# yanielc/medical-vision-textural-bias

Hardware: AMD Instinct MI355X
Metric: BraTS 4ch 240^3 vols/sec filtered+train-step @1/2/4/8 GPU; filter HBM GB/s (higher is better)
Workload: dtype f32

## Files before the change

medical-vision-textural-bias_amd/csrc/conv_up.hip:

```cpp
#include <hip/hip_runtime.h>

#include <cstdlib>
#include <type_traits>

#include "num_cu.h"
#include "texbias.h"

namespace {

typedef float f2v __attribute__((ext_vector_type(2)));
typedef float f32x4 __attribute__((ext_vector_type(4)));
typedef const __attribute__((address_space(4))) float* cfloat_p;
typedef const __attribute__((address_space(4))) f2v* cf2v_p;

template <int B, int N, class F>
__device__ __forceinline__ void static_for(F&& f) {
  if constexpr (B < N) {
    f(std::integral_constant<int, B>{});
    static_for<B + 1, N>(f);
  }
}

struct S2Args {
  const float* in;
  const float* K;
  const float* bias;
  float* out;
  int Do, Ho, Wo, Di, Hi, Wi;
  int ZS, zlen, nyb;
  int PX, RR;
};

template <int CIN, int MOUT, int TY, int WV, int NTH = 256>
__global__ __launch_bounds__(NTH) void k_conv_s2_fewin(S2Args a) {
  static_assert(MOUT % 2 == 0, "packed output pairs");
  constexpr int NHALF = NTH / 256, MP = MOUT / 2 / NHALF;
  constexpr int NR = 2 * TY + 1;
  extern __shared__ __attribute__((aligned(16))) float smem[];
  const int tid = (int)threadIdx.x;
  constexpr int PX = 4 * WV + 12, SS = CIN * NR * PX;
  float* ring = smem;
  for (int i = tid; i < 3 * SS; i += NTH) ring[i] = 0.f;
  int b = (int)blockIdx.x;
  const int zs = b % a.ZS;
  b /= a.ZS;
  const int yb = b % a.nyb, n = b / a.nyb;
  const int y0 = yb * TY;
  const int z0 = zs * a.zlen, z1 = min(a.Do, z0 + a.zlen);
  const int Di = a.Di, Hi = a.Hi, Wi = a.Wi;
  const int64_t iplane = (int64_t)Hi * Wi, iplane4 = iplane / 4;
  const float4* inb = reinterpret_cast<const float4*>(a.in + (int64_t)n * CIN * Di * iplane);
  const int W4 = Wi >> 2;
  constexpr int NL = (CIN * NR * WV + NTH - 1) / NTH;
  int gof[NL], lof[NL];
#pragma unroll
  for (int j = 0; j < NL; ++j) {
    const int i = tid + NTH * j;
    const int q = i % W4, t = i / W4, r = t % NR, c = t / NR;
    const int yi = 2 * y0 - 1 + r;
    const bool ok = c < CIN && yi >= 0 && yi < Hi;
    gof[j] = ok ? (int)((int64_t)c * Di * iplane4 + ((int64_t)yi * Wi + 4 * q) / 4) : -1;
    lof[j] = (c * NR + r) * PX + 4 + 4 * q;
  }
  float4 ra[NL], rb[NL];
  auto load = [&](int zi, float4 (&r)[NL]) {
    const bool in = zi >= 0 && zi < Di;
    const float4* src = inb + (int64_t)(in ? zi : 0) * iplane4;
#pragma unroll
    for (int j = 0; j < NL; ++j) {
      r[j] = src[gof[j] < 0 ? 0 : gof[j]];
    }
  };
  auto store = [&](int zi, const float4 (&r)[NL]) {
    float* d = ring + ((zi + 3) % 3) * SS;
    const bool in = zi >= 0 && zi < Di;
#pragma unroll
    for (int j = 0; j < NL; ++j)
      if (gof[j] >= 0) *reinterpret_cast<float4*>(d + lof[j]) = in ? r[j] : make_float4(0.f, 0.f, 0.f, 0.f);
  };
  __syncthreads();
  load(2 * z0 - 1, ra);
  store(2 * z0 - 1, ra);
  load(2 * z0, ra);
  load(2 * z0 + 1, rb);
  const int pt = tid & 255, mh = __builtin_amdgcn_readfirstlane(tid >> 8);
  const int Wo = a.Wo, oy = pt / Wo, ox = pt - oy * Wo;
  const bool act = oy < TY && y0 + oy < a.Ho;
  const int roff = (2 * oy) * PX + 2 * ox + 3;
  f2v bias2[MP];
#pragma unroll
  for (int mm = 0; mm < MP; ++mm) {
    const int m = mh * MP + mm;
    bias2[mm] = a.bias ? f2v{a.bias[2 * m], a.bias[2 * m + 1]} : f2v{0.f, 0.f};
  }
  const int64_t oplane = (int64_t)a.Ho * Wo;
  float* outb = a.out + (int64_t)n * MOUT * a.Do * oplane + (int64_t)(y0 + oy) * Wo + ox;
  constexpr bool LATE = NTH == 256;
  f2v pend[MP];
  auto put = [&](int zp) {
    float* o = outb + (int64_t)zp * oplane;
#pragma unroll
    for (int mm = 0; mm < MP; ++mm) {
      const int m = mh * MP + mm;
      o[(int64_t)(2 * m) * a.Do * oplane] = pend[mm].x;
      o[(int64_t)(2 * m + 1) * a.Do * oplane] = pend[mm].y;
    }
  };
  for (int z = z0; z < z1; ++z) {
    store(2 * z, ra);
    store(2 * z + 1, rb);
    __syncthreads();
    if (LATE || z + 1 < z1) {
      load(2 * z + 2, ra);
      load(2 * z + 3, rb);
    }
    if (LATE && act && z > z0) put(z - 1);
    if (act) {
      float v[CIN * 27];
#pragma unroll
      for (int tz = 0; tz < 3; ++tz) {
        const float* sl = ring + ((2 * z - 1 + tz + 3) % 3) * SS + roff;
#pragma unroll
        for (int c = 0; c < CIN; ++c)
#pragma unroll
          for (int ty = 0; ty < 3; ++ty)
#pragma unroll
            for (int tx = 0; tx < 3; ++tx) v[c * 27 + tz * 9 + ty * 3 + tx] = sl[(c * NR + ty) * PX + tx];
      }
      constexpr int KC = CIN * 27, NP = MP * KC, BT = 16, NB = (NP + BT - 1) / BT;
      const cf2v_p kp = (cf2v_p)(cfloat_p)a.K + mh * NP;
      f2v kb[2][BT];
      auto kload = [&](int b, f2v (&k)[BT]) {
#pragma unroll
        for (int i = 0; i < BT; ++i)
          if (b * BT + i < NP) k[i] = kp[b * BT + i];
      };
      kload(0, kb[0]);
      f2v acc = bias2[0];
      static_for<0, NB>([&](auto bc) {
        constexpr int b = decltype(bc)::value;
        __builtin_amdgcn_sched_barrier(0);
        __builtin_amdgcn_s_waitcnt(0xc07f);
        __builtin_amdgcn_sched_barrier(0);
        if (b + 1 < NB) kload(b + 1, kb[(b + 1) & 1]);
        __builtin_amdgcn_sched_barrier(0);
#pragma unroll
        for (int i = 0; i < BT; ++i) {
          const int p = b * BT + i, mm = p / KC, k = p - mm * KC;
          if (p < NP) {
            if (k == 0) acc = bias2[mm];
            acc = __builtin_elementwise_fma(f2v{v[k], v[k]}, kb[b & 1][i], acc);
            if (k == KC - 1) {
              if (LATE) {
                pend[mm] = acc;
              } else {
                const int m = mh * MP + mm;
                float* o = outb + (int64_t)z * oplane;
                o[(int64_t)(2 * m) * a.Do * oplane] = acc.x;
                o[(int64_t)(2 * m + 1) * a.Do * oplane] = acc.y;
              }
            }
          }
        }
      });
    }
    __syncthreads();
  }
  if (LATE && act && z1 > z0) put(z1 - 1);
}

struct TArgs {
  const float* x;
  const float* W;
  const float* bias;
  float* y;
  int Cin, Di, Hi, Wi;
  int ZS, zlen, nyb;
  int PX, CS;
};

template <int MO, int TY, int WV, int NTH = 256, int U = 1>
__global__ __launch_bounds__(NTH) void k_convT_fewout(TArgs a) {
  extern __shared__ __attribute__((aligned(16))) float smem[];
  const int tid = (int)threadIdx.x;
  constexpr int PX = 4 * WV + 8, CS = (TY + 1) * PX;
  const int Cin = a.Cin, SS = Cin * CS;
  float* ring = smem;
  for (int i = tid; i < 2 * SS; i += NTH) ring[i] = 0.f;
  const cfloat_p wg = (cfloat_p)a.W;
  int b = (int)blockIdx.x;
  const int zs = b % a.ZS;
  b /= a.ZS;
  const int yb = b % a.nyb, n = b / a.nyb;
  const int y0 = yb * TY;
  const int Di = a.Di, Hi = a.Hi, Wi = a.Wi;
  const int z0 = zs * a.zlen, z1 = min(Di, z0 + a.zlen);
  const int64_t iplane = (int64_t)Hi * Wi, iplane4 = iplane / 4;
  const float4* xb = reinterpret_cast<const float4*>(a.x + (int64_t)n * Cin * Di * iplane);
  const int W4 = Wi >> 2;
  constexpr int NL = (32 * (TY + 1) * WV + NTH - 1) / NTH;
  const int nitem = Cin * (TY + 1) * W4;
  int gof[NL], lof[NL];
#pragma unroll
  for (int j = 0; j < NL; ++j) {
    const int i = tid + NTH * j;
    const int q = i % W4, t = i / W4, r = t % (TY + 1), c = t / (TY + 1);
    const int yi = y0 + r;
    const bool ok = i < nitem && yi < Hi;
    gof[j] = ok ? (int)((int64_t)c * Di * iplane4 + ((int64_t)yi * Wi + 4 * q) / 4) : -1;
    lof[j] = c * CS + r * PX + 4 + 4 * q;
  }
  float4 rg[NL];
  auto load = [&](int zi) {
    const bool in = zi < Di;
    const float4* src = xb + (int64_t)(in ? zi : 0) * iplane4;
#pragma unroll
    for (int j = 0; j < NL; ++j) {
      rg[j] = src[gof[j] < 0 ? 0 : gof[j]];
    }
  };
  auto store = [&](int zi) {
    float* d = ring + (zi & 1) * SS;
    const bool in = zi < Di;
#pragma unroll
    for (int j = 0; j < NL; ++j)
      if (gof[j] >= 0) *reinterpret_cast<float4*>(d + lof[j]) = in ? rg[j] : make_float4(0.f, 0.f, 0.f, 0.f);
  };
  __syncthreads();
  load(z0);
  store(z0);
  load(z0 + 1);
  const int jy = tid / Wi, jx = tid - jy * Wi;
  const bool act = jy < TY && y0 + jy < Hi;
  const int roff = jy * PX + jx + 4;
  const int Ho = 2 * Hi, Wo = 2 * Wi, Do = 2 * Di;
  const int64_t oplane = (int64_t)Ho * Wo;
  float bia[MO];
#pragma unroll
  for (int m = 0; m < MO; ++m) bia[m] = a.bias ? a.bias[m] : 0.f;
  float* yb0 = a.y + (int64_t)n * MO * Do * oplane + (int64_t)(2 * (y0 + jy)) * Wo + 2 * jx;
  for (int z = z0; z < z1; ++z) {
    store(z + 1);
    __syncthreads();
    if (z + 1 < z1) load(z + 2);
    float acc[MO][2][2][2];
#pragma unroll
    for (int m = 0; m < MO; ++m)
#pragma unroll
      for (int p = 0; p < 8; ++p) acc[m][p >> 2][(p >> 1) & 1][p & 1] = bia[m];
    if (act) {
      const float* s0 = ring + (z & 1) * SS + roff;
      const float* s1 = ring + ((z + 1) & 1) * SS + roff;
#pragma unroll U
      for (int c = 0; c < Cin; ++c) {
        float v[2][2][2];
        v[0][0][0] = s0[c * CS];
        v[0][0][1] = s0[c * CS + 1];
        v[0][1][0] = s0[c * CS + PX];
        v[0][1][1] = s0[c * CS + PX + 1];
        v[1][0][0] = s1[c * CS];
        v[1][0][1] = s1[c * CS + 1];
        v[1][1][0] = s1[c * CS + PX];
        v[1][1][1] = s1[c * CS + PX + 1];
        const cfloat_p wc = wg + c * MO * 27;
#pragma unroll
        for (int m = 0; m < MO; ++m) {
          const cfloat_p wk = wc + m * 27;
#pragma unroll
          for (int pz = 0; pz < 2; ++pz)
#pragma unroll
            for (int py = 0; py < 2; ++py)
#pragma unroll
              for (int px = 0; px < 2; ++px) {
                float s = acc[m][pz][py][px];
#pragma unroll
                for (int dz = 0; dz <= pz; ++dz)
#pragma unroll
                  for (int dy = 0; dy <= py; ++dy)
#pragma unroll
                    for (int dx = 0; dx <= px; ++dx) {
                      const int tz = pz ? (dz ? 0 : 2) : 1, ty = py ? (dy ? 0 : 2) : 1, tx = px ? (dx ? 0 : 2) : 1;
                      s = fmaf(v[dz][dy][dx], wk[tz * 9 + ty * 3 + tx], s);
                    }
                acc[m][pz][py][px] = s;
              }
        }
      }
#pragma unroll
      for (int m = 0; m < MO; ++m)
#pragma unroll
        for (int pz = 0; pz < 2; ++pz)
#pragma unroll
          for (int py = 0; py < 2; ++py) {
            float* o = yb0 + ((int64_t)m * Do + 2 * z + pz) * oplane + (int64_t)py * Wo;
            *reinterpret_cast<float2*>(o) = make_float2(acc[m][pz][py][0], acc[m][pz][py][1]);
          }
    }
    __syncthreads();
  }
}

int zseg(int D, int base, int per_cu, int fill) {
  const int slots = per_cu * tb::num_cu();
  int best = 1 << 30, zl = D;
  for (int l = D; l >= 1; --l) {
    const int zs = (D + l - 1) / l, rounds = (base * zs + slots - 1) / slots, cost = rounds * (l + fill);
    if (cost < best) best = cost, zl = l;
  }
  return zl;
}

template <int CIN, int MOUT, int WV>
int launch_s2(S2Args& a, size_t lds, int N, hipStream_t st) {
  constexpr int TY = 3;
  constexpr int NT = (CIN == 4 && MOUT == 32) ? 512 : 256;
  auto kern = k_conv_s2_fewin<CIN, MOUT, TY, WV, NT>;
  if (hipFuncSetAttribute(reinterpret_cast<const void*>(kern), hipFuncAttributeMaxDynamicSharedMemorySize, 163840) !=
      hipSuccess)
    return TB_ERR_HIP;
  const int per_cu = lds <= 81920 ? 2 : 1;
  a.zlen = zseg(a.Do, N * a.nyb, per_cu, 1);
  a.ZS = (a.Do + a.zlen - 1) / a.zlen;
  hipLaunchKernelGGL(kern, dim3((unsigned)(N * a.nyb * a.ZS)), dim3(NT), lds, st, a);
  return hipGetLastError() == hipSuccess ? TB_OK : TB_ERR_HIP;
}

}

int tb_conv3d_s2_fewin_f32(const float* in, const float* K, const float* bias, float* out, int N, int Cin, int Mout,
                           int Do, int Ho, int Wo, void* stream) {
  if (!in || !K || !out || N < 1 || Do < 1 || Ho < 1 || Wo < 1) return TB_ERR_INVALID_ARG;
  if (Cin < 1 || Cin > 4 || (Mout != 16 && Mout != 32) || 3 * Wo > 256 || (2 * Wo) % 4 != 0 || 2 * Wo > 256 ||
      (reinterpret_cast<uintptr_t>(in) & 15) != 0)
    return TB_ERR_UNSUPPORTED_SIZE;
  constexpr int TY = 3;
  S2Args a{};
  a.in = in, a.K = K, a.bias = bias, a.out = out;
  a.Do = Do, a.Ho = Ho, a.Wo = Wo, a.Di = 2 * Do, a.Hi = 2 * Ho, a.Wi = 2 * Wo;
  const bool wide = a.Wi > 160;
  a.PX = 4 * (wide ? 64 : 40) + 12;
  a.RR = 2 * TY + 1;
  a.nyb = (Ho + TY - 1) / TY;
  const size_t lds = (size_t)4 * 3 * Cin * a.RR * a.PX;
  if (lds > 163840) return TB_ERR_UNSUPPORTED_SIZE;
  hipStream_t st = reinterpret_cast<hipStream_t>(stream);
#define TB_S2(CI, MO)                                                                                  \
  if (Cin == CI && Mout == MO) return wide ? launch_s2<CI, MO, 64>(a, lds, N, st) : launch_s2<CI, MO, 40>(a, lds, N, st);
  TB_S2(1, 16) TB_S2(2, 16) TB_S2(3, 16) TB_S2(4, 16) TB_S2(1, 32) TB_S2(2, 32) TB_S2(3, 32) TB_S2(4, 32)
#undef TB_S2
  return TB_ERR_UNSUPPORTED_SIZE;
}

int tb_convT3d_fewout_f32(const float* x, const float* W, const float* bias, float* y, int N, int Cin, int Mout, int Di,
                          int Hi, int Wi, void* stream) {
  if (!x || !W || !y || N < 1 || Di < 1 || Hi < 1 || Wi < 1) return TB_ERR_INVALID_ARG;
  if (Cin < 1 || Cin > 32 || Mout < 1 || Mout > 4 || Wi % 4 != 0 || Wi > 128 || (reinterpret_cast<uintptr_t>(x) & 15) != 0)
    return TB_ERR_UNSUPPORTED_SIZE;
  const bool big = Wi <= 80 && (size_t)4 * 2 * Cin * 7 * (4 * 20 + 8) <= 163840;
  const int TY = big ? 6 : 256 / Wi >= 3 ? 3 : 256 / Wi >= 2 ? 2 : 1;
  const int nth = big ? 512 : 256;
  TArgs a{};
  a.x = x, a.W = W, a.bias = bias, a.y = y;
  a.Cin = Cin, a.Di = Di, a.Hi = Hi, a.Wi = Wi;
  a.PX = 4 * (Wi <= 80 ? 20 : 32) + 8;
  a.CS = (TY + 1) * a.PX;
  a.nyb = (Hi + TY - 1) / TY;
  const size_t lds = (size_t)4 * 2 * Cin * a.CS;
  if (lds > 163840) return TB_ERR_UNSUPPORTED_SIZE;
  const int per_cu = lds <= 81920 ? 2 : 1;
  a.zlen = zseg(Di, N * a.nyb, per_cu, 1);
  a.ZS = (Di + a.zlen - 1) / a.zlen;
  hipStream_t st = reinterpret_cast<hipStream_t>(stream);
  const dim3 grid((unsigned)(N * a.nyb * a.ZS));
  void (*kern)(TArgs) = nullptr;
#define TB_T(MO, T)                                                                    \
  if (Mout == MO && TY == T) kern = Wi <= 80 ? k_convT_fewout<MO, T, 20> : k_convT_fewout<MO, T, 32>;
  TB_T(1, 1) TB_T(1, 2) TB_T(1, 3) TB_T(2, 1) TB_T(2, 2) TB_T(2, 3) TB_T(3, 1) TB_T(3, 2) TB_T(3, 3) TB_T(4, 1)
  TB_T(4, 2) TB_T(4, 3)
#undef TB_T
  constexpr int U = 1;
  if (big && Mout == 3)
    kern = U == 4 ? k_convT_fewout<3, 6, 20, 512, 4> : U == 2 ? k_convT_fewout<3, 6, 20, 512, 2>
                                                      : k_convT_fewout<3, 6, 20, 512>;
  else if (big)
    kern = Mout == 1 ? k_convT_fewout<1, 6, 20, 512> : Mout == 2 ? k_convT_fewout<2, 6, 20, 512>
                                                     : k_convT_fewout<4, 6, 20, 512>;
  if (!kern) return TB_ERR_UNSUPPORTED_SIZE;
  if (hipFuncSetAttribute(reinterpret_cast<const void*>(kern), hipFuncAttributeMaxDynamicSharedMemorySize, 163840) !=
      hipSuccess)
    return TB_ERR_HIP;
  hipLaunchKernelGGL(kern, grid, dim3(nth), lds, st, a);
  return hipGetLastError() == hipSuccess ? TB_OK : TB_ERR_HIP;
}

namespace {
struct F16Args {
  const float* x;
  const float* W;
  const float* bias;
  const float* add;
  float* y;
  int D, H, Wd;
  int ZS, zlen, nyb;
  int PX, RX;
  int flip;
  int persist, ncol;
  int64_t addsn;
};

template <int YB, int NXT, int NTH, bool ADD = false, bool PF = false, int NS = 3>
__global__ __launch_bounds__(NTH) void k_conv3d_fwd16(F16Args a) {
  constexpr int NWV = NTH / 64;
  extern __shared__ __attribute__((aligned(16))) float smem[];
  constexpr int NR = YB + 2, W4 = 4 * NXT;
  const int tid = (int)threadIdx.x, lane = tid & 63;
  const int wave = __builtin_amdgcn_readfirstlane(tid >> 6);
  const int D = a.D, H = a.H, Wd = a.Wd, PX = a.PX, RX = a.RX, SS = 16 * RX;
  float* ring = smem;
  for (int i = tid; i < NS * SS; i += NTH) ring[i] = 0.f;
  const int li = lane & 15, ks = lane >> 4;
  float af[108];
#pragma unroll
  for (int kk = 0; kk < 108; ++kk) {
    const int c = 4 * (kk & 3) + ks, t = kk >> 2;
    af[kk] = a.flip ? a.W[(c * 16 + li) * 27 + 26 - t] : a.W[(li * 16 + c) * 27 + t];
  }
  const float bm[4] = {a.bias ? a.bias[4 * ks] : 0.f, a.bias ? a.bias[4 * ks + 1] : 0.f,
                       a.bias ? a.bias[4 * ks + 2] : 0.f, a.bias ? a.bias[4 * ks + 3] : 0.f};
  int64_t s_beg, s_end;
  if (a.persist) {
    const int64_t T = (int64_t)a.ncol * D;
    s_beg = T * blockIdx.x / gridDim.x, s_end = T * (blockIdx.x + 1) / gridDim.x;
  } else {
    int b = (int)blockIdx.x;
    const int zs = b % a.ZS;
    b /= a.ZS;
    const int zb = zs * a.zlen;
    s_beg = (int64_t)b * D + zb, s_end = (int64_t)b * D + min(D, zb + a.zlen);
  }
  for (int64_t sg = s_beg; sg < s_end;) {
  const int col = (int)(sg / D), z0 = (int)(sg - (int64_t)col * D);
  const int z1 = (int)min((int64_t)D, z0 + (s_end - sg));
  sg += z1 - z0;
  const int yb = col % a.nyb, n = col / a.nyb;
  const int y0 = yb * YB;
  const int64_t plane = (int64_t)H * Wd, plane4 = plane / 4;
  const float4* xb = reinterpret_cast<const float4*>(a.x + (int64_t)n * 16 * D * plane);
  constexpr int NL = (16 * NR * W4 + NTH - 1) / NTH;
  int gof[NL], lof[NL];
#pragma unroll
  for (int j = 0; j < NL; ++j) {
    const int i = tid + NTH * j;
    const int q = i % W4, t = i / W4, r = t % NR, c = t / NR;
    const int yi = y0 - 1 + r;
    const bool ok = i < 16 * NR * W4 && yi >= 0 && yi < H;
    gof[j] = ok ? (int)((int64_t)c * D * plane4 + ((int64_t)yi * Wd + 4 * q) / 4) : -1;
    lof[j] = i < 16 * NR * W4 ? c * RX + r * PX + 4 + 4 * q : 0;
  }
  float4 rg[NL];
  auto load = [&](int zi) {
    const bool in = zi >= 0 && zi < D;
    const float4* src = xb + (int64_t)(in ? zi : 0) * plane4;
#pragma unroll
    for (int j = 0; j < NL; ++j) {
      rg[j] = src[gof[j] < 0 ? 0 : gof[j]];
    }
  };
  auto store = [&](int zi) {
    float* d = ring + ((zi + NS) % NS) * SS;
    const bool in = zi >= 0 && zi < D;
#pragma unroll
    for (int j = 0; j < NL; ++j)
      *reinterpret_cast<float4*>(d + lof[j]) = in && gof[j] >= 0 ? rg[j] : make_float4(0.f, 0.f, 0.f, 0.f);
  };
  __syncthreads();
  load(z0 - 1);
  store(z0 - 1);
  load(z0);
  store(z0);
  load(z0 + 1);
  store(z0 + 1);
  __builtin_amdgcn_s_waitcnt(0x0F70);
  __syncthreads();
  const int bl = ks * RX + li + 3;
  const int64_t oplane = plane;
  float* yb0 = a.y + (int64_t)n * 16 * D * oplane;
  const float* ab0 = ADD ? a.add + (int64_t)n * (a.addsn ? a.addsn : 16 * D * oplane) : nullptr;
  constexpr int NT = YB * NXT;
  constexpr int NIT = (NT + 2 * NWV - 1) / (2 * NWV);
  for (int z = z0; z < z1; ++z) {
    const bool more = z + 1 < z1;
    if (more) load(z + 2);
    float av[NIT][2][4];
    if constexpr (ADD) {
#pragma unroll
      for (int it = 0; it < NIT; ++it) {
        const int t0 = wave + 2 * NWV * it;
        if (t0 >= NT) break;
        const int t1 = t0 + NWV < NT ? t0 + NWV : t0;
        const int yy0 = t0 / NXT, x00 = 16 * (t0 - yy0 * NXT);
        const int yy1 = t1 / NXT, x01 = 16 * (t1 - yy1 * NXT);
        const int ya = min(y0 + yy0, H - 1), yc = min(y0 + yy1, H - 1);
#pragma unroll
        for (int r = 0; r < 4; ++r) {
          const int m = 4 * ks + r;
          av[it][0][r] = ab0[((int64_t)m * D + z) * oplane + (int64_t)ya * Wd + x00 + li];
          av[it][1][r] = ab0[((int64_t)m * D + z) * oplane + (int64_t)yc * Wd + x01 + li];
        }
      }
    }
    const float* s0 = ring + ((z + NS - 1) % NS) * SS + bl;
    const float* s1 = ring + (z % NS) * SS + bl;
    const float* s2 = ring + ((z + 1) % NS) * SS + bl;
    f32x4 acc[NIT][2];
#pragma unroll
    for (int it = 0; it < NIT; ++it) {
      const int t0 = wave + 2 * NWV * it;
      if (t0 >= NT) break;
      const int t1 = t0 + NWV < NT ? t0 + NWV : t0;
      const int yy0 = t0 / NXT, x00 = 16 * (t0 - yy0 * NXT);
      const int yy1 = t1 / NXT, x01 = 16 * (t1 - yy1 * NXT);
      const int o0 = yy0 * PX + x00, o1 = yy1 * PX + x01;
      f32x4 acc0 = {bm[0], bm[1], bm[2], bm[3]}, acc1 = acc0;
      if constexpr (PF) {
        float bq[2][8];
        auto ldb = [&](int t, float (&q)[8]) {
          const int tz = t / 9, ty = (t / 3) % 3, tx = t % 3;
          const float* sl = tz == 0 ? s0 : tz == 1 ? s1 : s2;
#pragma unroll
          for (int cq = 0; cq < 4; ++cq) {
            const int off = 4 * cq * RX + ty * PX + tx;
            q[2 * cq] = sl[o0 + off], q[2 * cq + 1] = sl[o1 + off];
          }
        };
        ldb(0, bq[0]);
#pragma unroll
        for (int t = 0; t < 27; ++t) {
          if (t + 1 < 27) ldb(t + 1, bq[(t + 1) & 1]);
#pragma unroll
          for (int cq = 0; cq < 4; ++cq) {
            acc0 = __builtin_amdgcn_mfma_f32_16x16x4f32(af[4 * t + cq], bq[t & 1][2 * cq], acc0, 0, 0, 0);
            acc1 = __builtin_amdgcn_mfma_f32_16x16x4f32(af[4 * t + cq], bq[t & 1][2 * cq + 1], acc1, 0, 0, 0);
          }
        }
#pragma unroll
        for (int i = 0; i < 216; ++i) {
          __builtin_amdgcn_sched_group_barrier(0x008, 1, 0);
          __builtin_amdgcn_sched_group_barrier(0x100, 1, 0);
        }
      } else {
#pragma unroll
      for (int tz = 0; tz < 3; ++tz) {
        const float* sl = tz == 0 ? s0 : tz == 1 ? s1 : s2;
#pragma unroll
        for (int ty = 0; ty < 3; ++ty)
#pragma unroll
          for (int tx = 0; tx < 3; ++tx) {
            const int t = tz * 9 + ty * 3 + tx;
#pragma unroll
            for (int cq = 0; cq < 4; ++cq) {
              const int off = 4 * cq * RX + ty * PX + tx;
              const float b0 = sl[o0 + off], b1 = sl[o1 + off];
              acc0 = __builtin_amdgcn_mfma_f32_16x16x4f32(af[4 * t + cq], b0, acc0, 0, 0, 0);
              acc1 = __builtin_amdgcn_mfma_f32_16x16x4f32(af[4 * t + cq], b1, acc1, 0, 0, 0);
            }
          }
      }
      }
      acc[it][0] = acc0, acc[it][1] = acc1;
    }
    if constexpr (NS == 3) __syncthreads();
    store(z + 2);
#pragma unroll
    for (int it = 0; it < NIT; ++it) {
      const int t0 = wave + 2 * NWV * it;
      if (t0 >= NT) break;
      const int t1 = t0 + NWV < NT ? t0 + NWV : t0;
      const int yy0 = t0 / NXT, x00 = 16 * (t0 - yy0 * NXT);
      const int yy1 = t1 / NXT, x01 = 16 * (t1 - yy1 * NXT);
#pragma unroll
      for (int r = 0; r < 4; ++r) {
        const int m = 4 * ks + r;
        const int64_t o0 = ((int64_t)m * D + z) * oplane + (int64_t)(y0 + yy0) * Wd + x00 + li;
        const int64_t o1 = ((int64_t)m * D + z) * oplane + (int64_t)(y0 + yy1) * Wd + x01 + li;
        if (y0 + yy0 < H) yb0[o0] = ADD ? acc[it][0][r] + av[it][0][r] : acc[it][0][r];
        if (t1 != t0 && y0 + yy1 < H) yb0[o1] = ADD ? acc[it][1][r] + av[it][1][r] : acc[it][1][r];
      }
    }
    __syncthreads();
  }
  }
}
}



int tb_conv3d_fwd16_f32(const float* x, const float* W, const float* bias, float* y, int N, int D, int H, int Wd,
                        void* stream) {
  return tb_conv3d_fwd16_add_f32(x, W, bias, nullptr, y, N, D, H, Wd, stream);
}

static int fwd16_call(const float* x, const float* W, const float* bias, const float* add, float* y, int N, int D, int H,
                      int Wd, int flip, void* stream, int64_t add_sn = 0);

int tb_conv3d_fwd16_add_f32(const float* x, const float* W, const float* bias, const float* add, float* y, int N, int D,
                            int H, int Wd, void* stream) {
  return fwd16_call(x, W, bias, add, y, N, D, H, Wd, 0, stream);
}

int tb_conv3d_fwd16_dgrad_f32(const float* gy, const float* W, const float* add, int64_t add_sn, float* dx, int N, int D,
                              int H, int Wd, void* stream) {
  return fwd16_call(gy, W, nullptr, add, dx, N, D, H, Wd, 1, stream, add_sn);
}

static int fwd16_call(const float* x, const float* W, const float* bias, const float* add, float* y, int N, int D, int H,
                      int Wd, int flip, void* stream, int64_t add_sn) {
  if (!x || !W || !y || N < 1 || D < 1 || H < 1 || Wd < 1) return TB_ERR_INVALID_ARG;
  if (Wd % 16 != 0 || Wd > 128 || (reinterpret_cast<uintptr_t>(x) & 15) != 0) return TB_ERR_UNSUPPORTED_SIZE;
  constexpr int YB = 3;
  F16Args a{};
  a.x = x, a.W = W, a.bias = bias, a.add = add, a.y = y, a.D = D, a.H = H, a.Wd = Wd;
  a.flip = flip;
  a.addsn = add_sn;
  a.PX = Wd + 8;
  a.RX = (YB + 2) * a.PX;
  while ((a.RX & 31) != 16) ++a.RX;
  a.nyb = (H + YB - 1) / YB;
  const int NS = (size_t)4 * 4 * 16 * a.RX <= 163840 ? 4 : 3;
  const size_t lds = (size_t)NS * 4 * 16 * a.RX;
  if (lds > 163840) return TB_ERR_UNSUPPORTED_SIZE;
  const int per_cu = 163840 / (int)lds >= 2 ? 2 : 1;
  a.zlen = zseg(D, N * a.nyb, per_cu, 2);
  a.ZS = (D + a.zlen - 1) / a.zlen;
  void (*kern)(F16Args) = nullptr;
  constexpr int NTv = 512;
  constexpr bool PFv = true;
  if (PFv && YB == 3 && NTv == 512 && Wd == 80) {
    kern = add ? (NS == 4 ? k_conv3d_fwd16<3, 5, 512, true, true, 4> : k_conv3d_fwd16<3, 5, 512, true, true, 3>)
               : (NS == 4 ? k_conv3d_fwd16<3, 5, 512, false, true, 4> : k_conv3d_fwd16<3, 5, 512, false, true, 3>);
  } else
#define TB_F16C(Y, X, T) \
  kern = add ? (NS == 4 ? k_conv3d_fwd16<Y, X, T, true, false, 4> : k_conv3d_fwd16<Y, X, T, true, false, 3>) \
             : (NS == 4 ? k_conv3d_fwd16<Y, X, T, false, false, 4> : k_conv3d_fwd16<Y, X, T, false, false, 3>);
#define TB_F16(Y, T)                                                                                   \
  if (YB == Y && NTv == T) switch (Wd / 16) {                                                          \
      case 1: TB_F16C(Y, 1, T) break;                                                                  \
      case 2: TB_F16C(Y, 2, T) break;                                                                  \
      case 3: TB_F16C(Y, 3, T) break;                                                                  \
      case 4: TB_F16C(Y, 4, T) break;                                                                  \
      case 5: TB_F16C(Y, 5, T) break;                                                                  \
      case 6: TB_F16C(Y, 6, T) break;                                                                  \
      case 7: TB_F16C(Y, 7, T) break;                                                                  \
      case 8: TB_F16C(Y, 8, T) break;                                                                  \
      default: return TB_ERR_UNSUPPORTED_SIZE;                                                         \
    }
  TB_F16(3, 512)
#undef TB_F16
#undef TB_F16C
  if (hipFuncSetAttribute(reinterpret_cast<const void*>(kern), hipFuncAttributeMaxDynamicSharedMemorySize, 163840) !=
      hipSuccess)
    return TB_ERR_HIP;
  constexpr int persist_env = 1;
  a.ncol = N * a.nyb;
  unsigned nblk = (unsigned)(N * a.nyb * a.ZS);
  a.persist = persist_env && per_cu == 1 && (int64_t)a.ncol * D >= 8LL * tb::num_cu() && nblk % tb::num_cu() != 0;
  if (a.persist) nblk = (unsigned)tb::num_cu();
  hipLaunchKernelGGL(kern, dim3(nblk), dim3(NTv), lds, reinterpret_cast<hipStream_t>(stream), a);
  return hipGetLastError() == hipSuccess ? TB_OK : TB_ERR_HIP;
}

namespace {
struct T64Args {
  const float* x;
  const float* W;
  const float* bias;
  float* y;
  int Di, Hi, Wi;
  int ZS, zlen, nyb;
  int PX, RX;
};

template <int G, int YB, int NL>
__global__ __launch_bounds__(256) void k_convT_mfma64(T64Args a) {
  extern __shared__ __attribute__((aligned(16))) float smem[];
  constexpr int NR = YB + 1;
  constexpr int CIN = 16 * G, HT = 4 / G;
  const int tid = (int)threadIdx.x, lane = tid & 63;
  const int w = __builtin_amdgcn_readfirstlane(tid >> 6);
  const int g = w % G, h = w / G;
  const int Di = a.Di, Hi = a.Hi, Wi = a.Wi, PX = a.PX, RX = a.RX, SS = CIN * RX;
  float* ring = smem;
  float* part = smem + 2 * SS;
  for (int i = tid; i < 2 * SS; i += 256) ring[i] = 0.f;
  int b = (int)blockIdx.x;
  const int zs = b % a.ZS;
  b /= a.ZS;
  const int yb = b % a.nyb, n = b / a.nyb;
  const int y0 = yb * YB;
  const int z0 = zs * a.zlen, z1 = min(Di, z0 + a.zlen);
  const int li = lane & 15, ks = lane >> 4;
  float af[108];
#pragma unroll
  for (int kk = 0; kk < 108; ++kk) af[kk] = a.W[((16 * g + 4 * (kk & 3) + ks) * 16 + li) * 27 + (kk >> 2)];
  const int64_t plane = (int64_t)Hi * Wi;
  const float* xb = a.x + (int64_t)n * CIN * Di * plane;
  const int W4 = Wi >> 2, per_c = NR * W4, total = CIN * per_c;
  const int64_t cstride = (int64_t)Di * plane;
  int gof[NL], lof[NL], gch[NL];
#pragma unroll
  for (int j = 0; j < NL; ++j) {
    const int i = tid + 256 * j;
    const int c = i / per_c, r2 = i - c * per_c, r = r2 / W4, q = r2 - r * W4;
    const int yi = y0 + r;
    lof[j] = i < total ? c * RX + r * PX + 4 * q : Wi;
    gof[j] = (i < total && yi < Hi) ? yi * Wi + 4 * q : -1;
    gch[j] = i < total ? c : 0;
  }
  float4 rg[NL];
  auto load = [&](int zi) {
    const bool in = zi < Di;
    const float* src = xb + (int64_t)(in ? zi : 0) * plane;
#pragma unroll
    for (int j = 0; j < NL; ++j) {
      const bool ok = in && gof[j] >= 0;
      rg[j] = *reinterpret_cast<const float4*>(src + gch[j] * cstride + (ok ? gof[j] : 0));
    }
  };
  auto store = [&](int zi) {
    float* d = ring + (zi & 1) * SS;
    const bool in = zi < Di;
#pragma unroll
    for (int j = 0; j < NL; ++j)
      *reinterpret_cast<float4*>(d + lof[j]) = (in && gof[j] >= 0) ? rg[j] : make_float4(0.f, 0.f, 0.f, 0.f);
  };
  float bm[4];
#pragma unroll
  for (int r = 0; r < 4; ++r) bm[r] = a.bias ? a.bias[4 * ks + r] : 0.f;
  __syncthreads();
  load(z0);
  store(z0);
  load(z0 + 1);
  store(z0 + 1);
  __builtin_amdgcn_s_waitcnt(0x0F70);
  __syncthreads();
  const int npos = YB * Wi, ntile = (npos + 15) / 16;
  const int64_t oplane = 4 * plane, orow = 2 * Wi;
  float* yb0 = a.y + (int64_t)n * 16 * (2 * Di) * oplane;
  auto sums = [&](int z, int t0, int pb) {
    const float* pr = part + pb * 4 * 8 * 256;
    for (int k = w; k < 4 * HT; k += 4) {
      const int hq = k >> 2, pz = (k >> 1) & 1, py = k & 1, q0 = pz * 4 + py * 2;
      const int pq = 16 * (t0 + hq) + li, yq = pq / Wi, xq = pq - yq * Wi;
      const bool okp = t0 + hq < ntile && pq < npos && y0 + yq < Hi;
#pragma unroll
      for (int r = 0; r < 4; ++r) {
        const int m = 4 * ks + r, e = m * 16 + li;
        float v0 = bm[r], v1 = bm[r];
#pragma unroll
        for (int v = 0; v < G; ++v) {
          v0 += pr[((hq * G + v) * 8 + q0) * 256 + e];
          v1 += pr[((hq * G + v) * 8 + q0 + 1) * 256 + e];
        }
        if (okp)
          *reinterpret_cast<float2*>(yb0 + ((int64_t)m * (2 * Di) + 2 * z + pz) * oplane +
                                     (int64_t)(2 * (y0 + yq) + py) * orow + 2 * xq) = make_float2(v0, v1);
      }
    }
  };
  int buf = 0;
  for (int z = z0; z < z1; ++z) {
    if (z + 1 < z1) load(z + 2);
    const float* sz[2] = {ring + (z & 1) * SS, ring + ((z + 1) & 1) * SS};
    for (int t0 = 0; t0 < ntile; t0 += HT) {
      const int tI = t0 + h;
      const int p = 16 * tI + li, pc = p < npos ? p : npos - 1;
      const int yy = pc / Wi, xx = pc - yy * Wi;
      const int bl = (16 * g + ks) * RX + yy * PX + xx;
      f32x4 acc[8];
#pragma unroll
      for (int q = 0; q < 8; ++q) acc[q] = f32x4{0.f, 0.f, 0.f, 0.f};
#pragma unroll
      for (int tz = 0; tz < 3; ++tz)
#pragma unroll
        for (int ty = 0; ty < 3; ++ty)
#pragma unroll
          for (int tx = 0; tx < 3; ++tx) {
            const int t = tz * 9 + ty * 3 + tx;
            const int par = (tz != 1) * 4 + (ty != 1) * 2 + (tx != 1);
            const float* s = sz[tz == 0] + bl + (ty == 0) * PX + (tx == 0);
#pragma unroll
            for (int cq = 0; cq < 4; ++cq)
              acc[par] = __builtin_amdgcn_mfma_f32_16x16x4f32(af[4 * t + cq], s[4 * cq * RX], acc[par], 0, 0, 0);
          }
      float* pw = part + (buf * 4 + w) * 8 * 256;
#pragma unroll
      for (int q = 0; q < 8; ++q)
#pragma unroll
        for (int r = 0; r < 4; ++r) pw[q * 256 + (4 * ks + r) * 16 + li] = acc[q][r];
      __syncthreads();
      if (t0 > 0) sums(z, t0 - HT, buf ^ 1);
      buf ^= 1;
    }
    store(z + 2);
    sums(z, ((ntile - 1) / HT) * HT, buf ^ 1);
    __syncthreads();
  }
}
}

int tb_convT3d_mfma64_f32(const float* x, const float* W, const float* bias, float* y, int N, int Di, int Hi, int Wi,
                          void* stream) {
  return tb_convT3d_mfma_f32(x, W, bias, y, N, 64, Di, Hi, Wi, stream);
}

int tb_convT3d_mfma_f32(const float* x, const float* W, const float* bias, float* y, int N, int Cin, int Di, int Hi,
                        int Wi, void* stream) {
  if (!x || !W || !y || N < 1 || Di < 1 || Hi < 1 || Wi < 1) return TB_ERR_INVALID_ARG;
  if (Cin != 32 && Cin != 64) return TB_ERR_UNSUPPORTED_SIZE;
  if (Wi % 4 != 0 || Wi > 64 || (reinterpret_cast<uintptr_t>(x) & 15) != 0 || (reinterpret_cast<uintptr_t>(y) & 7) != 0)
    return TB_ERR_UNSUPPORTED_SIZE;
  constexpr int YB = 2;
  T64Args a{};
  a.x = x, a.W = W, a.bias = bias, a.y = y, a.Di = Di, a.Hi = Hi, a.Wi = Wi;
  a.PX = Wi + 4;
  a.RX = (YB + 1) * a.PX;
  while ((a.RX & 31) != 16) ++a.RX;
  a.nyb = (Hi + YB - 1) / YB;
  const size_t lds = (size_t)4 * (2 * Cin * a.RX + 2 * 4 * 8 * 256);
  if (lds > 163840) return TB_ERR_UNSUPPORTED_SIZE;
  a.zlen = zseg(Di, N * a.nyb, 1, 1);
  a.ZS = (Di + a.zlen - 1) / a.zlen;
  const int nl = (Cin * (YB + 1) * (Wi / 4) + 255) / 256;
  void (*kern)(T64Args) = nullptr;
  switch (nl) {
#define TB_NL(k) \
  case k: kern = Cin == 64 ? k_convT_mfma64<4, YB, k> : k_convT_mfma64<2, YB, k>; break;
    TB_NL(1) TB_NL(2) TB_NL(3) TB_NL(4) TB_NL(5) TB_NL(6) TB_NL(7) TB_NL(8) TB_NL(9) TB_NL(10) TB_NL(11) TB_NL(12)
#undef TB_NL
    default: return TB_ERR_UNSUPPORTED_SIZE;
  }
  if (hipFuncSetAttribute(reinterpret_cast<const void*>(kern), hipFuncAttributeMaxDynamicSharedMemorySize, 163840) !=
      hipSuccess)
    return TB_ERR_HIP;
  hipLaunchKernelGGL(kern, dim3((unsigned)(N * a.nyb * a.ZS)), dim3(256), lds, reinterpret_cast<hipStream_t>(stream), a);
  return hipGetLastError() == hipSuccess ? TB_OK : TB_ERR_HIP;
}

namespace {
struct S1Args {
  const float* x;
  const float* W;
  const float* bias;
  const float* add;
  float* y;
  int D, H, Wd, YB;
  int ZS, zlen, nyb, MG;
  int PX, RX;
  int flip;
  int64_t addsn;
};

template <int G, int NC, int NL, int NTH, bool ADD = false>
__global__ __launch_bounds__(NTH) void k_conv3d_mfma_s1(S1Args a) {
  constexpr int CIN = 16 * G, MTB = 4 / G, NWG = NTH / 256;
  extern __shared__ __attribute__((aligned(16))) float smem[];
  const int tid = (int)threadIdx.x, lane = tid & 63;
  const int w = __builtin_amdgcn_readfirstlane(tid >> 6);
  const int g = w % G, mt = (w / G) % MTB, h = w / 4;
  const int D = a.D, H = a.H, Wd = a.Wd, YB = a.YB, PX = a.PX, RX = a.RX, SS = CIN * RX;
  const int NR = YB + 2;
  float* ring = smem;
  float* part = smem + 3 * SS;
  float* bsm = part + (NTH / 64) * NC * 256;
  for (int i = tid; i < 3 * SS; i += NTH) ring[i] = 0.f;
  int b = (int)blockIdx.x;
  const int zs = b % a.ZS;
  b /= a.ZS;
  const int mg = b % a.MG;
  b /= a.MG;
  const int yb = b % a.nyb, n = b / a.nyb;
  const int COUT = 16 * MTB * a.MG;
  const int y0 = yb * YB;
  const int z0 = zs * a.zlen, z1 = min(D, z0 + a.zlen);
  const int li = lane & 15, ks = lane >> 4;
  const int m0 = (mg * MTB + mt) * 16;
  if (tid < MTB * 16) bsm[tid] = a.bias ? a.bias[mg * MTB * 16 + tid] : 0.f;
  float af[108];
#pragma unroll
  for (int kk = 0; kk < 108; ++kk) {
    const int c = 16 * g + 4 * (kk & 3) + ks, t = kk >> 2;
    af[kk] = a.flip ? a.W[(c * CIN + m0 + li) * 27 + 26 - t] : a.W[((m0 + li) * CIN + c) * 27 + t];
  }
  const int64_t plane = (int64_t)H * Wd, cstride = (int64_t)D * plane;
  const float* xb = a.x + (int64_t)n * CIN * cstride;
  const int W4 = Wd >> 2, per_c = NR * W4, total = CIN * per_c;
  int gof[NL], lof[NL], gch[NL];
#pragma unroll
  for (int j = 0; j < NL; ++j) {
    const int i = tid + NTH * j;
    const int c = i / per_c, r2 = i - c * per_c, r = r2 / W4, q = r2 - r * W4;
    const int yi = y0 - 1 + r;
    lof[j] = i < total ? c * RX + r * PX + 4 + 4 * q : 0;
    gof[j] = (i < total && yi >= 0 && yi < H) ? yi * Wd + 4 * q : -1;
    gch[j] = i < total ? c : 0;
  }
  float4 rg[NL];
  auto load = [&](int zi) {
    const bool in = zi >= 0 && zi < D;
    const float* src = xb + (int64_t)(in ? zi : 0) * plane;
#pragma unroll
    for (int j = 0; j < NL; ++j) {
      const bool ok = in && gof[j] >= 0;
      rg[j] = *reinterpret_cast<const float4*>(src + gch[j] * cstride + (ok ? gof[j] : 0));
    }
  };
  auto store = [&](int zi) {
    float* d = ring + ((zi + 3) % 3) * SS;
    const bool in = zi >= 0 && zi < D;
#pragma unroll
    for (int j = 0; j < NL; ++j)
      *reinterpret_cast<float4*>(d + lof[j]) = (in && gof[j] >= 0) ? rg[j] : make_float4(0.f, 0.f, 0.f, 0.f);
  };
  __syncthreads();
  load(z0 - 1);
  store(z0 - 1);
  load(z0);
  store(z0);
  load(z0 + 1);
  store(z0 + 1);
  __builtin_amdgcn_s_waitcnt(0x0F70);
  __syncthreads();
  const int npos = YB * Wd;
  float* ybase = a.y + (int64_t)n * COUT * cstride;
  const float* abase = ADD ? a.add + (int64_t)n * (a.addsn ? a.addsn : COUT * cstride) : nullptr;
  constexpr int NK = (MTB * NWG * NC + NTH / 64 - 1) / (NTH / 64);
  int bl[NC];
#pragma unroll
  for (int c = 0; c < NC; ++c) {
    const int p = 16 * (NWG * c + h) + li, pc = p < npos ? p : npos - 1;
    const int yy = pc / Wd, xx = pc - yy * Wd;
    bl[c] = (16 * g + ks) * RX + yy * PX + xx + 3;
  }
  for (int z = z0; z < z1; ++z) {
    if (z + 1 < z1) load(z + 2);
    float av[NK][4];
    if constexpr (ADD) {
#pragma unroll
      for (int kk = 0; kk < NK; ++kk) {
        const int k = w + kk * (NTH / 64);
        if (k >= MTB * NWG * NC) break;
        const int mq = k / (NWG * NC), r2 = k - mq * (NWG * NC), hq = r2 / NC, c = r2 - hq * NC;
        const int p = 16 * (NWG * c + hq) + li, pc = p < npos ? p : npos - 1;
        const int yy = pc / Wd, xx = pc - yy * Wd, yr = min(y0 + yy, H - 1);
        const int mb = (mg * MTB + mq) * 16;
#pragma unroll
        for (int r = 0; r < 4; ++r)
          av[kk][r] = abase[(int64_t)(mb + 4 * ks + r) * cstride + (int64_t)z * plane + (int64_t)yr * Wd + xx];
      }
    }
    const float* sp[3] = {ring + ((z + 2) % 3) * SS, ring + (z % 3) * SS, ring + ((z + 1) % 3) * SS};
    f32x4 acc[NC];
#pragma unroll
    for (int c = 0; c < NC; ++c) acc[c] = f32x4{0.f, 0.f, 0.f, 0.f};
#pragma unroll
    for (int tz = 0; tz < 3; ++tz)
#pragma unroll
      for (int ty = 0; ty < 3; ++ty)
#pragma unroll
        for (int tx = 0; tx < 3; ++tx) {
          const int t = tz * 9 + ty * 3 + tx;
          const float* s = sp[tz] + ty * PX + tx;
#pragma unroll
          for (int cq = 0; cq < 4; ++cq)
#pragma unroll
            for (int c = 0; c < NC; ++c)
              acc[c] = __builtin_amdgcn_mfma_f32_16x16x4f32(af[4 * t + cq], s[bl[c] + 4 * cq * RX], acc[c], 0, 0, 0);
        }
    float* pw = part + w * NC * 256;
#pragma unroll
    for (int c = 0; c < NC; ++c)
#pragma unroll
      for (int r = 0; r < 4; ++r) pw[c * 256 + (4 * ks + r) * 16 + li] = acc[c][r];
    __syncthreads();
    store(z + 2);
    auto combo = [&](int k, int kk) {
      const int mq = k / (NWG * NC), r2 = k - mq * (NWG * NC), hq = r2 / NC, c = r2 - hq * NC;
      const int p = 16 * (NWG * c + hq) + li;
      const int yy = p / Wd, xx = p - yy * Wd;
      const bool ok = p < npos && y0 + yy < H;
      const int mb = (mg * MTB + mq) * 16;
#pragma unroll
      for (int r = 0; r < 4; ++r) {
        const int m = 4 * ks + r;
        float v = bsm[mq * 16 + m];
#pragma unroll
        for (int gg = 0; gg < G; ++gg) v += part[((hq * 4 + mq * G + gg) * NC + c) * 256 + m * 16 + li];
        const int64_t o = (int64_t)(mb + m) * cstride + (int64_t)z * plane + (int64_t)(y0 + yy) * Wd + xx;
        if (ok) ybase[o] = ADD ? v + av[kk][r] : v;
      }
    };
    if constexpr (ADD) {
#pragma unroll
      for (int kk = 0; kk < NK; ++kk) {
        const int k = w + kk * (NTH / 64);
        if (k >= MTB * NWG * NC) break;
        combo(k, kk);
      }
    } else {
      for (int k = w; k < MTB * NWG * NC; k += NTH / 64) combo(k, 0);
    }
    __syncthreads();
  }
}
}

int tb_conv3d_mfma_f32(const float* x, const float* W, const float* bias, float* y, int N, int C, int D, int H, int Wd,
                       void* stream) {
  return tb_conv3d_mfma_add_f32(x, W, bias, nullptr, y, N, C, D, H, Wd, stream);
}

static int mfma_call(const float* x, const float* W, const float* bias, const float* add, float* y, int N, int C, int D,
                     int H, int Wd, int flip, void* stream, int64_t add_sn = 0);

int tb_conv3d_mfma_add_f32(const float* x, const float* W, const float* bias, const float* add, float* y, int N, int C,
                           int D, int H, int Wd, void* stream) {
  return mfma_call(x, W, bias, add, y, N, C, D, H, Wd, 0, stream);
}

int tb_conv3d_mfma_dgrad_f32(const float* gy, const float* W, const float* add, int64_t add_sn, float* dx, int N, int C,
                             int D, int H, int Wd, void* stream) {
  return mfma_call(gy, W, nullptr, add, dx, N, C, D, H, Wd, 1, stream, add_sn);
}

static int mfma_call(const float* x, const float* W, const float* bias, const float* add, float* y, int N, int C, int D,
                     int H, int Wd, int flip, void* stream, int64_t add_sn) {
  if (!x || !W || !y || N < 1 || D < 1 || H < 1 || Wd < 1) return TB_ERR_INVALID_ARG;
  if ((C != 32 && C != 64) || Wd % 4 != 0 || Wd > 64 || (reinterpret_cast<uintptr_t>(x) & 15) != 0)
    return TB_ERR_UNSUPPORTED_SIZE;
  constexpr int NTv = 256;
  const int NC = NTv == 512 ? 3 : 5;
  const int G = C / 16;
  S1Args a{};
  a.x = x, a.W = W, a.bias = bias, a.add = add, a.y = y, a.D = D, a.H = H, a.Wd = Wd;
  a.flip = flip;
  a.addsn = add_sn;
  a.PX = Wd + 8;
  a.MG = G == 2 ? 1 : 4;
  size_t lds = 0;
  int YB = std::max(1, 16 * NC * (NTv / 256) / Wd);
  for (; YB >= 1; --YB) {
    a.RX = (YB + 2) * a.PX;
    while ((a.RX & 31) != 16) ++a.RX;
    lds = (size_t)4 * (3 * C * a.RX + (NTv / 64) * NC * 256 + 64);
    if (lds <= 163840) break;
  }
  if (YB < 1) return TB_ERR_UNSUPPORTED_SIZE;
  a.YB = YB > H ? H : YB;
  a.nyb = (H + a.YB - 1) / a.YB;
  a.zlen = zseg(D, N * a.nyb * a.MG, 1, 2);
  a.ZS = (D + a.zlen - 1) / a.zlen;
  const int nl = (C * (a.YB + 2) * (Wd / 4) + NTv - 1) / NTv;
  void (*kern)(S1Args) = nullptr;
#define TB_NL(k)                                                                                      \
  case k:                                                                                             \
    kern = add ? (G == 2 ? k_conv3d_mfma_s1<2, 5, k, 256, true> : k_conv3d_mfma_s1<4, 5, k, 256, true>) \
               : (G == 2 ? k_conv3d_mfma_s1<2, 5, k, 256> : k_conv3d_mfma_s1<4, 5, k, 256>);             \
    break;
  switch (nl) {
    TB_NL(1) TB_NL(2) TB_NL(3) TB_NL(4) TB_NL(5) TB_NL(6) TB_NL(7) TB_NL(8) TB_NL(9) TB_NL(10) TB_NL(11) TB_NL(12)
    default: return TB_ERR_UNSUPPORTED_SIZE;
  }
#undef TB_NL
  if (hipFuncSetAttribute(reinterpret_cast<const void*>(kern), hipFuncAttributeMaxDynamicSharedMemorySize, 163840) !=
      hipSuccess)
    return TB_ERR_HIP;
  hipLaunchKernelGGL(kern, dim3((unsigned)(N * a.nyb * a.MG * a.ZS)), dim3(NTv), lds,
                     reinterpret_cast<hipStream_t>(stream), a);
  return hipGetLastError() == hipSuccess ? TB_OK : TB_ERR_HIP;
}
```

Measured before the change: 174.1.

## Route 16-channel conv3d through split-bf16 MFMA kernel with persistent scheduling

Adds a new 16-channel 3x3x3 conv kernel that splits each f32 operand into three bf16 parts and emulates f32 accumulation with six bf16 MFMA 16x16x32 products. Input z-planes are staged in an LDS ring buffer in pre-split form. Weights are held in registers. Launch becomes persistent when the block count does not divide evenly by the CU count. The aim is to use the bf16 matrix cores instead of the previous f32 path, at the cost of extra split arithmetic, three times the LDS footprint, and a possible small loss of precision versus true f32.

```diff
diff --git a/medical-vision-textural-bias_amd/csrc/conv_up.hip b/medical-vision-textural-bias_amd/csrc/conv_up.hip
--- a/medical-vision-textural-bias_amd/csrc/conv_up.hip
+++ b/medical-vision-textural-bias_amd/csrc/conv_up.hip
@@ -4,6 +4,7 @@
 #include <type_traits>
 
 #include "num_cu.h"
+#include "split_bf16.h"
 #include "texbias.h"
 
 namespace {
@@ -594,6 +595,200 @@
 }
 
 
+namespace {
+struct X16Args {
+  const float* x;
+  const float* W;
+  const float* bias;
+  const float* add;
+  float* y;
+  int D, H, Wd;
+  int ZS, zlen, nyb;
+  int flip;
+  int persist, ncol;
+  int64_t addsn;
+};
+
+constexpr int x16_pxp(int W) { return W + 5; }
+constexpr size_t x16_slot(int W) { return (size_t)3 * 5 * x16_pxp(W) * 32; }
+
+template <int NXT, bool ADD, int NS>
+__global__ __launch_bounds__(512) void k_conv16_split(X16Args a) {
+  using tb::bf16x8;
+  constexpr int YB = 3, NR = YB + 2, NTH = 512, NWV = NTH / 64, W = 16 * NXT, W4 = 4 * NXT;
+  constexpr int RPB = x16_pxp(W) * 32, SPL = NR * RPB, SLOT = 3 * SPL;
+  constexpr int NTASK = 4 * NR * W4;
+  static_assert(NTASK <= NTH && 2 * SPL + RPB < 65536 && (size_t)SLOT == x16_slot(W), "one task per thread");
+  extern __shared__ __attribute__((aligned(16))) char ring16[];
+  const int tid = (int)threadIdx.x, lane = tid & 63;
+  const int wave = __builtin_amdgcn_readfirstlane(tid >> 6);
+  const int D = a.D, H = a.H;
+  for (int i = tid; i < NS * SLOT / 16; i += NTH) reinterpret_cast<uint4*>(ring16)[i] = make_uint4(0, 0, 0, 0);
+  const int li = lane & 15, g = lane >> 4, hi = g >> 1;
+  bf16x8 af[14][3];
+  const int wsm = a.flip ? 27 : 16 * 27, wsc = a.flip ? 16 * 27 : 27;
+  const float* wl = a.W + li * wsm + 8 * (g & 1) * wsc;
+#pragma unroll
+  for (int q = 0; q < 14; ++q) {
+    const int t = 2 * q + hi, tc = t < 27 ? t : 26;
+    const float* wq = wl + (a.flip ? 26 - tc : tc);
+    float v[8];
+#pragma unroll
+    for (int j = 0; j < 8; ++j) v[j] = wq[j * wsc];
+    if (q == 13) {
+#pragma unroll
+      for (int j = 0; j < 8; ++j) v[j] = hi ? 0.f : v[j];
+    }
+    tb::split3(v, af[q][0], af[q][1], af[q][2]);
+  }
+  const float bm[4] = {a.bias ? a.bias[4 * g] : 0.f, a.bias ? a.bias[4 * g + 1] : 0.f,
+                       a.bias ? a.bias[4 * g + 2] : 0.f, a.bias ? a.bias[4 * g + 3] : 0.f};
+  int64_t s_beg, s_end;
+  if (a.persist) {
+    const int64_t T = (int64_t)a.ncol * D;
+    s_beg = T * blockIdx.x / gridDim.x, s_end = T * (blockIdx.x + 1) / gridDim.x;
+  } else {
+    int b = (int)blockIdx.x;
+    const int zs = b % a.ZS;
+    b /= a.ZS;
+    const int zb = zs * a.zlen;
+    s_beg = (int64_t)b * D + zb, s_end = (int64_t)b * D + min(D, zb + a.zlen);
+  }
+  const bool act = tid < NTASK;
+  const int cq = tid & 3, rr = act ? (tid >> 2) % NR : 0, q4 = act ? (tid >> 2) / NR : 0;
+  const int lof = act ? rr * RPB + (4 * q4 + 1) * 32 + cq * 8 : (W + 1) * 32;
+  const int lb = li * 32 + 16 * (g & 1);
+  constexpr int NT = YB * NXT;
+  constexpr int NIT = (NT + NWV - 1) / NWV;
+  for (int64_t sg = s_beg; sg < s_end;) {
+    const int col = (int)(sg / D), z0 = (int)(sg - (int64_t)col * D);
+    const int z1 = (int)min((int64_t)D, z0 + (s_end - sg));
+    sg += z1 - z0;
+    const int yb = col % a.nyb, n = col / a.nyb;
+    const int y0 = yb * YB;
+    const int64_t plane = (int64_t)H * W, plane4 = plane / 4, chq = (int64_t)D * plane4;
+    const float4* xb = reinterpret_cast<const float4*>(a.x + (int64_t)n * 16 * D * plane);
+    const int yi = y0 - 1 + rr;
+    const bool rowok = act && yi >= 0 && yi < H;
+    const unsigned gof = rowok ? (unsigned)(16 * (4 * cq * chq) + 4 * ((int64_t)yi * W + 4 * q4)) : 0u;
+    const unsigned lo = (unsigned)(4 * ((int64_t)4 * g * D * plane + li));
+    float4 rg[4];
+    auto load = [&](int zi) {
+      const char* src = reinterpret_cast<const char*>(xb + (int64_t)(zi < 0 ? 0 : zi >= D ? D - 1 : zi) * plane4);
+#pragma unroll
+      for (int c = 0; c < 4; ++c) rg[c] = *reinterpret_cast<const float4*>(src + 16 * c * chq + gof);
+    };
+    auto store = [&](int zi) {
+      char* d = ring16 + ((zi + NS) % NS) * SLOT + lof;
+      const unsigned m = 0u - (unsigned)(rowok && zi >= 0 && zi < D);
+#pragma unroll
+      for (int e = 0; e < 4; ++e) {
+        float v[4];
+#pragma unroll
+        for (int c = 0; c < 4; ++c)
+          v[c] = __uint_as_float(__float_as_uint(e == 0 ? rg[c].x : e == 1 ? rg[c].y : e == 2 ? rg[c].z : rg[c].w) & m);
+        unsigned p[3][2];
+        tb::split3_pk(v[0], v[1], p[0][0], p[1][0], p[2][0]);
+        tb::split3_pk(v[2], v[3], p[0][1], p[1][1], p[2][1]);
+#pragma unroll
+        for (int s = 0; s < 3; ++s) *reinterpret_cast<uint2*>(d + s * SPL + e * 32) = make_uint2(p[s][0], p[s][1]);
+      }
+    };
+    __syncthreads();
+    load(z0 - 1);
+    store(z0 - 1);
+    load(z0);
+    store(z0);
+    load(z0 + 1);
+    store(z0 + 1);
+    __builtin_amdgcn_s_waitcnt(0x0F70);
+    __syncthreads();
+    float* yb0 = a.y + (int64_t)n * 16 * D * plane;
+    const float* ab0 = ADD ? a.add + (int64_t)n * (a.addsn ? a.addsn : 16 * D * plane) : nullptr;
+    for (int z = z0; z < z1; ++z) {
+      load(z + 2);
+      int hv = hi;
+      asm volatile("" : "+v"(hv));
+      int sb[3];
+#pragma unroll
+      for (int tz = 0; tz < 3; ++tz) sb[tz] = ((z + tz + NS - 1) % NS) * SLOT;
+      tb::f32x4s cl = {0.f, 0.f, 0.f, 0.f};
+      float avl[4] = {0.f, 0.f, 0.f, 0.f};
+#pragma unroll
+      for (int it = 0; it < NIT; ++it) {
+        const int t = wave + NWV * it;
+        if (t < NT) {
+          const int yy = t / NXT, x0 = 16 * (t - yy * NXT);
+          const int64_t ou = ((int64_t)z * plane + (int64_t)min(y0 + yy, H - 1) * W + x0) * 4;
+          float av[4];
+          if constexpr (ADD) {
+#pragma unroll
+            for (int r = 0; r < 4; ++r)
+              av[r] = *reinterpret_cast<const float*>(reinterpret_cast<const char*>(ab0) + ou + 4 * r * D * plane + lo);
+          }
+          const char* rb = ring16 + yy * RPB + x0 * 32 + lb;
+          bf16x8 bq[2][3];
+          auto ldb = [&](int q, bf16x8 (&b)[3]) {
+            const int t0 = 2 * q, t1 = 2 * q + 1 < 27 ? 2 * q + 1 : 26;
+            const int c0 = ((t0 / 3) % 3) * RPB + (t0 % 3) * 32, c1 = ((t1 / 3) % 3) * RPB + (t1 % 3) * 32;
+            const int o = t0 / 9 == t1 / 9 ? sb[t0 / 9] + (hv ? c1 : c0) : hv ? sb[t1 / 9] + c1 : sb[t0 / 9] + c0;
+            b[1] = *reinterpret_cast<const bf16x8*>(rb + o + SPL);
+            b[2] = *reinterpret_cast<const bf16x8*>(rb + o + 2 * SPL);
+            b[0] = *reinterpret_cast<const bf16x8*>(rb + o);
+          };
+          tb::f32x4s c = {0.f, 0.f, 0.f, 0.f}, cs = c;
+          ldb(0, bq[0]);
+#pragma unroll
+          for (int q = 0; q < 14; ++q) {
+            if (q + 1 < 14) ldb(q + 1, bq[(q + 1) & 1]);
+            tb::mfma_split6(af[q], bq[q & 1], c, cs);
+          }
+          c += cs;
+#pragma unroll
+          for (int r = 0; r < 4; ++r) c[r] += bm[r];
+          if constexpr (ADD) __builtin_amdgcn_sched_group_barrier(0x020, 4, 0);
+          __builtin_amdgcn_sched_group_barrier(0x100, 3, 0);
+#pragma unroll
+          for (int q = 0; q < 13; ++q) {
+            __builtin_amdgcn_sched_group_barrier(0x100, 3, 0);
+            __builtin_amdgcn_sched_group_barrier(0x008, 6, 0);
+          }
+          __builtin_amdgcn_sched_group_barrier(0x008, 6, 0);
+          if constexpr (ADD) {
+#pragma unroll
+            for (int r = 0; r < 4; ++r) asm volatile("" : "+v"(av[r]));
+          }
+          if (it == NIT - 1) {
+            cl = c;
+            if constexpr (ADD) {
+#pragma unroll
+              for (int r = 0; r < 4; ++r) avl[r] = av[r];
+            }
+          } else if (y0 + yy < H) {
+#pragma unroll
+            for (int r = 0; r < 4; ++r)
+              *reinterpret_cast<float*>(reinterpret_cast<char*>(yb0) + ou + 4 * r * D * plane + lo) = ADD ? c[r] + av[r] : c[r];
+          }
+        }
+      }
+      if constexpr (NS == 3) __syncthreads();
+      store(z + 2);
+      {
+        const int t = wave + NWV * (NIT - 1);
+        const int yy = t / NXT, x0 = 16 * (t - yy * NXT);
+        if (t < NT && y0 + yy < H) {
+          const int64_t ou = ((int64_t)z * plane + (int64_t)(y0 + yy) * W + x0) * 4;
+#pragma unroll
+          for (int r = 0; r < 4; ++r)
+            *reinterpret_cast<float*>(reinterpret_cast<char*>(yb0) + ou + 4 * r * D * plane + lo) = ADD ? cl[r] + avl[r] : cl[r];
+        }
+      }
+      __syncthreads();
+    }
+  }
+}
+}
+
 
 int tb_conv3d_fwd16_f32(const float* x, const float* W, const float* bias, float* y, int N, int D, int H, int Wd,
                         void* stream) {
@@ -611,12 +806,44 @@
 int tb_conv3d_fwd16_dgrad_f32(const float* gy, const float* W, const float* add, int64_t add_sn, float* dx, int N, int D,
                               int H, int Wd, void* stream) {
   return fwd16_call(gy, W, nullptr, add, dx, N, D, H, Wd, 1, stream, add_sn);
+}
+
+static int split16_call(const float* x, const float* W, const float* bias, const float* add, float* y, int N, int D,
+                        int H, int Wd, int flip, void* stream, int64_t add_sn) {
+  X16Args a{};
+  a.x = x, a.W = W, a.bias = bias, a.add = add, a.y = y, a.D = D, a.H = H, a.Wd = Wd;
+  a.flip = flip;
+  a.addsn = add_sn;
+  a.nyb = (H + 2) / 3;
+  const int NS = 4 * x16_slot(Wd) <= 163840 ? 4 : 3;
+  const size_t lds = NS * x16_slot(Wd);
+  a.zlen = zseg(D, N * a.nyb, 1, 2);
+  a.ZS = (D + a.zlen - 1) / a.zlen;
+  void (*kern)(X16Args) = nullptr;
+#define TB_X16(NX, S) \
+  case NX: kern = add ? k_conv16_split<NX, true, S> : k_conv16_split<NX, false, S>; break;
+  switch (Wd / 16) {
+    TB_X16(1, 4) TB_X16(2, 4) TB_X16(3, 4) TB_X16(4, 4) TB_X16(5, 4) TB_X16(6, 3)
+    default: return TB_ERR_UNSUPPORTED_SIZE;
+  }
+#undef TB_X16
+  if (NS != (Wd <= 80 ? 4 : 3)) return TB_ERR_UNSUPPORTED_SIZE;
+  if (hipFuncSetAttribute(reinterpret_cast<const void*>(kern), hipFuncAttributeMaxDynamicSharedMemorySize, 163840) !=
+      hipSuccess)
+    return TB_ERR_HIP;
+  a.ncol = N * a.nyb;
+  unsigned nblk = (unsigned)(N * a.nyb * a.ZS);
+  a.persist = (int64_t)a.ncol * D >= 8LL * tb::num_cu() && nblk % tb::num_cu() != 0;
+  if (a.persist) nblk = (unsigned)tb::num_cu();
+  hipLaunchKernelGGL(kern, dim3(nblk), dim3(512), lds, reinterpret_cast<hipStream_t>(stream), a);
+  return hipGetLastError() == hipSuccess ? TB_OK : TB_ERR_HIP;
 }
 
 static int fwd16_call(const float* x, const float* W, const float* bias, const float* add, float* y, int N, int D, int H,
                       int Wd, int flip, void* stream, int64_t add_sn) {
   if (!x || !W || !y || N < 1 || D < 1 || H < 1 || Wd < 1) return TB_ERR_INVALID_ARG;
   if (Wd % 16 != 0 || Wd > 128 || (reinterpret_cast<uintptr_t>(x) & 15) != 0) return TB_ERR_UNSUPPORTED_SIZE;
+  if (3 * x16_slot(Wd) <= 163840 && (int64_t)16 * D * H * Wd < (1LL << 29)) return split16_call(x, W, bias, add, y, N, D, H, Wd, flip, stream, add_sn);
   constexpr int YB = 3;
   F16Args a{};
   a.x = x, a.W = W, a.bias = bias, a.add = add, a.y = y, a.D = D, a.H = H, a.Wd = Wd;
diff --git a/medical-vision-textural-bias_amd/csrc/split_bf16.h b/medical-vision-textural-bias_amd/csrc/split_bf16.h
--- /dev/null
+++ b/medical-vision-textural-bias_amd/csrc/split_bf16.h
@@ -0,0 +1,43 @@
+#pragma once
+#include <hip/hip_runtime.h>
+
+namespace tb {
+
+typedef __bf16 bf16x8 __attribute__((ext_vector_type(8)));
+typedef __bf16 bf16x2 __attribute__((ext_vector_type(2)));
+typedef float f32x2s __attribute__((ext_vector_type(2)));
+typedef float f32x4s __attribute__((ext_vector_type(4)));
+
+__device__ __forceinline__ void split3_pk(float a, float b, unsigned& p0, unsigned& p1, unsigned& p2) {
+  const float top = __uint_as_float(0x7f7f7fffu);
+  const bf16x2 h = __builtin_convertvector(
+      f32x2s{__builtin_amdgcn_fmed3f(a, -top, top), __builtin_amdgcn_fmed3f(b, -top, top)}, bf16x2);
+  p0 = __builtin_bit_cast(unsigned, h);
+  const float ra = a - __uint_as_float(p0 << 16), rb = b - __uint_as_float(p0 & 0xffff0000u);
+  const bf16x2 m = __builtin_convertvector(f32x2s{ra, rb}, bf16x2);
+  p1 = __builtin_bit_cast(unsigned, m);
+  const float sa = ra - __uint_as_float(p1 << 16), sb = rb - __uint_as_float(p1 & 0xffff0000u);
+  const bf16x2 l = __builtin_convertvector(f32x2s{sa, sb}, bf16x2);
+  p2 = __builtin_bit_cast(unsigned, l);
+}
+
+__device__ __forceinline__ void split3(const float (&v)[8], bf16x8& p0, bf16x8& p1, bf16x8& p2) {
+  unsigned q[3][4];
+#pragma unroll
+  for (int j = 0; j < 4; ++j) split3_pk(v[2 * j], v[2 * j + 1], q[0][j], q[1][j], q[2][j]);
+  typedef unsigned u32x4 __attribute__((ext_vector_type(4)));
+  p0 = __builtin_bit_cast(bf16x8, u32x4{q[0][0], q[0][1], q[0][2], q[0][3]});
+  p1 = __builtin_bit_cast(bf16x8, u32x4{q[1][0], q[1][1], q[1][2], q[1][3]});
+  p2 = __builtin_bit_cast(bf16x8, u32x4{q[2][0], q[2][1], q[2][2], q[2][3]});
+}
+
+__device__ __forceinline__ void mfma_split6(const bf16x8 (&a)[3], const bf16x8 (&b)[3], f32x4s& hi, f32x4s& lo) {
+  lo = __builtin_amdgcn_mfma_f32_16x16x32_bf16(a[1], b[1], lo, 0, 0, 0);
+  lo = __builtin_amdgcn_mfma_f32_16x16x32_bf16(a[0], b[2], lo, 0, 0, 0);
+  lo = __builtin_amdgcn_mfma_f32_16x16x32_bf16(a[2], b[0], lo, 0, 0, 0);
+  lo = __builtin_amdgcn_mfma_f32_16x16x32_bf16(a[0], b[1], lo, 0, 0, 0);
+  lo = __builtin_amdgcn_mfma_f32_16x16x32_bf16(a[1], b[0], lo, 0, 0, 0);
+  hi = __builtin_amdgcn_mfma_f32_16x16x32_bf16(a[0], b[0], hi, 0, 0, 0);
+}
+
+}
```

Result: faster. 183.2 (median of 6 runs) (+5.2%).
